# samtools/htslib

Hardware: NVIDIA H100
Metric: BGZF inflate + CRAM rANS decode GB/s at 1/2/4/8 H100 vs reference CPU (higher is better)
Workload: dtype u8

## Files before the change

### htslib_b200/csrc/bgzf_inflate.cu

```cuda
#include "hgpu_internal.h"

namespace {

constexpr int LIT_ROOT = 9, DST_ROOT = 8;
constexpr int LIT_TABLE = (1 << LIT_ROOT) + 856;
constexpr int DST_TABLE = (1 << DST_ROOT) + 512;
constexpr int CL_TABLE = 128;

enum : uint32_t { K_BAD = 0, K_LIT = 1, K_LEN = 2, K_SUB = 3, K_DIST = 4, K_EOB = 8 };
#define ENTRY(value, xb, kind, nbits) (((uint32_t)(value) << 16) | ((uint32_t)(xb) << 8) | ((uint32_t)(kind) << 4) | (uint32_t)(nbits))
constexpr uint32_t BAD_ENTRY = ENTRY(0, 0, K_BAD, 0);

struct InflateSmem {
    uint32_t lit[LIT_TABLE];
    uint32_t dst[DST_TABLE];
    union {
        struct {
            uint32_t cl[CL_TABLE];
            uint16_t code[320];
            uint8_t  lens[320];
            uint32_t count[16];
            uint32_t next[16];
            uint32_t sub_alloc;
        };
// ... 55 lines not shown
        b.w++;
        b.buf = v >> (8 * mis);
        b.cnt = 32 - 8 * (int)mis;
        b.avail -= b.cnt;
    }
}

__device__ __forceinline__ void bits_fill(Bits &b)
{
    if (b.cnt <= 32) {
        uint32_t v = b.w < b.wend ? (*b.w) : 0;
        b.w++;
        b.buf |= (uint64_t)v << b.cnt;
        b.cnt += 32;
        b.avail -= 32;
    }
}
__device__ __forceinline__ uint32_t bits_peek(const Bits &b, int n) { return (uint32_t)b.buf & ((1u << n) - 1u); }
__device__ __forceinline__ void bits_drop(Bits &b, int n) { b.buf >>= n; b.cnt -= n; }
__device__ __forceinline__ uint32_t bits_get(Bits &b, int n) { uint32_t v = bits_peek(b, n); bits_drop(b, n); return v; }
__device__ __forceinline__ bool bits_overrun(const Bits &b) { return b.avail + b.cnt < 0; }
__device__ __forceinline__ uint32_t bits_pos(const Bits &b) { return (uint32_t)((int64_t)b.end_bits - (b.avail + b.cnt)); }

template <int ROOT, int CAP, typename MakeEntry>
__device__ int build_table(InflateSmem &s, uint32_t *table, int n, bool allow_single, MakeEntry make)
{
    const uint32_t lane = hgpu_lane();
    __syncwarp();
    if (lane < 16) s.count[lane] = 0;
    for (int i = lane; i < CAP; i += 32) table[i] = BAD_ENTRY;
    if (lane == 0) s.sub_alloc = 1u << ROOT;
    __syncwarp();
    for (int i = lane; i < n; i += 32) atomicAdd(&s.count[s.lens[i]], 1u);
    __syncwarp();
    int maxlen = 0;
    int64_t left = 1;
    uint32_t code = 0;
    bool over = false;
    for (int l = 1; l <= 15; l++) {
        uint32_t c = s.count[l];
        left = (left << 1) - (int64_t)c;
        if (left < 0) over = true;
        if (c) maxlen = l;
        code = (code + (l > 1 ? s.count[l - 1] : 0)) << 1;
        if (l == 1) code = 0;
        if (lane == 0) s.next[l] = code;
    }
    if (over) return -1;
    if (maxlen == 0) return allow_single ? 0 : -1;
    if (left > 0 && !(allow_single && maxlen == 1)) return -1;
    __syncwarp();
    for (int base = 0; base < n; base += 32) {
        int i = base + lane;
        uint32_t l = i < n ? s.lens[i] : 0;
        uint32_t peers = __match_any_sync(0xffffffffu, l);
        uint32_t rank = __popc(peers & hgpu_lanemask_lt());
        if (l) s.code[i] = (uint16_t)(s.next[l] + rank);
        __syncwarp();
        if (l && rank + 1 == (uint32_t)__popc(peers)) s.next[l] += __popc(peers);
        __syncwarp();
    }
    for (int i = lane; i < n; i += 32) {
        uint32_t l = s.lens[i];
        if (!l) continue;
        uint32_t rev = __brev((uint32_t)s.code[i]) >> (32 - l);
        if (l <= ROOT) {
            uint32_t e = make(i, l);
            for (uint32_t k = rev; k < (1u << ROOT); k += 1u << l) table[k] = e;
        } else {
            atomicMax(&table[rev & ((1u << ROOT) - 1)], ENTRY(0, l - ROOT, K_SUB, ROOT) | 0x80000000u);
        }
    }
    __syncwarp();
    for (uint32_t k = lane; k < (1u << ROOT); k += 32) {
        uint32_t e = table[k];
        if (e & 0x80000000u) {
            uint32_t sub_bits = (e >> 8) & 0xff;
            uint32_t off = atomicAdd(&s.sub_alloc, 1u << sub_bits);
            table[k] = off + (1u << sub_bits) <= (uint32_t)CAP ? ENTRY(off, sub_bits, K_SUB, ROOT) : BAD_ENTRY;
        }
    }
    __syncwarp();
    if (s.sub_alloc > (uint32_t)CAP) return -1;
    for (int i = lane; i < n; i += 32) {
        uint32_t l = s.lens[i];
        if (l <= ROOT) continue;
        uint32_t rev = __brev((uint32_t)s.code[i]) >> (32 - l);
        uint32_t root = table[rev & ((1u << ROOT) - 1)];
        uint32_t off = root >> 16, sub_bits = (root >> 8) & 0xff;
        uint32_t e = make(i, l - ROOT);
        for (uint32_t k = rev >> ROOT; k < (1u << sub_bits); k += 1u << (l - ROOT)) table[off + k] = e;
    }
    __syncwarp();
    return 0;
}

__device__ __forceinline__ uint32_t lit_entry(int sym, uint32_t nbits)
{
    if (sym < 256) return ENTRY(sym, 0, K_LIT, nbits);
    if (sym == 256) return ENTRY(0, 0, K_EOB, nbits);
    if (sym > 285) return ENTRY(0, 0, K_BAD, nbits);
    return ENTRY(c_len_base[sym - 257], c_len_xtra[sym - 257], K_LEN, nbits);
}
__device__ __forceinline__ uint32_t dst_entry(int sym, uint32_t nbits)
{
    if (sym > 29) return ENTRY(0, 0, K_BAD, nbits);
    return ENTRY(c_dst_base[sym], c_dst_xtra[sym], K_DIST, nbits);
}
__device__ __forceinline__ uint32_t cl_entry(int sym, uint32_t nbits) { return ENTRY(sym, 0, K_LIT, nbits); }

template <int ROOT>
__device__ __forceinline__ uint32_t lookup(const uint32_t *table, Bits &b)
{
    uint32_t e = table[bits_peek(b, ROOT)];
    if (((e >> 4) & 15) == K_SUB) {
        bits_drop(b, ROOT);
        e = table[(e >> 16) + bits_peek(b, (e >> 8) & 0xff)];
    }
    bits_drop(b, e & 15);
    return e;
}

__device__ uint32_t multmodp(uint32_t a, uint32_t b)
{
    uint32_t p = 0;
    for (uint32_t m = 1u << 31; m; m >>= 1) {
        if (a & m) p ^= b;
        b = (b & 1) ? (b >> 1) ^ 0xEDB88320u : b >> 1;
    }
    return p;
}

__device__ uint32_t xpow_bytes(uint32_t nbytes)
{
    uint32_t p = 1u << 31;
    uint32_t sq = 1u << 23;
    while (nbytes) {
        if (nbytes & 1) p = multmodp(sq, p);
        sq = multmodp(sq, sq);
        nbytes >>= 1;
    }
    return p;
}

__global__ void crc_init_kernel()
{
    uint32_t i = threadIdx.x;
    uint32_t c = i;
    for (int k = 0; k < 8; k++) c = (c >> 1) ^ (0xEDB88320u & (0u - (c & 1)));
    g_crc_tab[0][i] = c;
    __syncthreads();
    uint32_t c1 = g_crc_tab[0][c & 0xff] ^ (c >> 8);
    g_crc_tab[1][i] = c1;
    uint32_t c2 = g_crc_tab[0][c1 & 0xff] ^ (c1 >> 8);
    g_crc_tab[2][i] = c2;
    uint32_t c3 = g_crc_tab[0][c2 & 0xff] ^ (c2 >> 8);
    g_crc_tab[3][i] = c3;
}

__global__ void crc_init2_kernel()
{
    const uint32_t i = threadIdx.x;
    for (int j = 0; j < 4; j++) {
        uint32_t v = g_crc_tab[j][i];
        for (int k = 0; k < 124; k++) v = g_crc_tab[0][v & 0xff] ^ (v >> 8);
        g_crc_tab2[j][i] = v;
    }
    g_xpow_lo[i] = xpow_bytes(i);
    g_xpow_hi[i] = xpow_bytes(256u * i);
    uint32_t v = 1u << 31;
    for (uint32_t k = 0; k < 8u * i; k++) v = (v & 0x80000000u) ? ((v ^ 0xEDB88320u) << 1) | 1u : v << 1;
    g_xinv_byte[i] = v;
}

__device__ uint32_t warp_crc32(const uint32_t (*tab)[256], const uint8_t *out, uint32_t n)
{
    const uint32_t lane = hgpu_lane();
    uint32_t c = n / 32, r = n % 32;
    uint32_t beg = lane == 0 ? 0 : r + lane * c;
    uint32_t len = lane == 0 ? c + r : c;
    uint32_t crc = 0xffffffffu;
    const uint8_t *p = out + beg, *e = p + len;
    while (p < e && (reinterpret_cast<uintptr_t>(p) & 15)) crc = tab[0][(crc ^ *p++) & 0xff] ^ (crc >> 8);
    if (e - p >= 16) {
        uint4 nx = *reinterpret_cast<const uint4 *>(p);
        while (e - p >= 16) {
            uint4 cur = nx;
            p += 16;
            if (e - p >= 16) nx = *reinterpret_cast<const uint4 *>(p);
            uint32_t wv[4] = {cur.x, cur.y, cur.z, cur.w};
#pragma unroll
            for (int k = 0; k < 4; k++) {
                crc ^= wv[k];
                crc = tab[3][crc & 0xff] ^ tab[2][(crc >> 8) & 0xff] ^ tab[1][(crc >> 16) & 0xff] ^ tab[0][crc >> 24];
            }
        }
    }
    while (p < e) crc = tab[0][(crc ^ *p++) & 0xff] ^ (crc >> 8);
    crc = ~crc;
    if (c == 0) return __shfl_sync(0xffffffffu, crc, 0);
    uint32_t xp = c < 65536u ? multmodp(g_xpow_hi[c >> 8], g_xpow_lo[c & 255u]) : xpow_bytes(c);
    for (int d = 1; d < 32; d <<= 1) {
        uint32_t right = __shfl_down_sync(0xffffffffu, crc, d);
        if ((lane & (2 * d - 1)) == 0) crc = multmodp(xp, crc) ^ right;
        xp = multmodp(xp, xp);
    }
    return __shfl_sync(0xffffffffu, crc, 0);
}

__device__ __forceinline__ uint32_t ld32_if(const uint8_t *a, bool c)
{
    uint32_t v;
    asm volatile("{\n\t.reg .pred q;\n\tsetp.ne.u32 q, %2, 0;\n\tmov.u32 %0, 0;\n\t@q ld.global.u32 %0, [%1];\n\t}" : "=r"(v) : "l"(a), "r"((uint32_t)c) : "memory");
    return v;
}
__device__ __forceinline__ void st32_if(uint8_t *a, uint32_t v, bool c)
{
    asm volatile("{\n\t.reg .pred q;\n\tsetp.ne.u32 q, %2, 0;\n\t@q st.global.u32 [%0], %1;\n\t}" :: "l"(a), "r"(v), "r"((uint32_t)c) : "memory");
}
__device__ __forceinline__ void st8_if(uint8_t *a, uint32_t v, bool c)
{
    asm volatile("{\n\t.reg .pred q;\n\tsetp.ne.u32 q, %2, 0;\n\t@q st.global.u8 [%0], %1;\n\t}" :: "l"(a), "r"(v), "r"((uint32_t)c) : "memory");
}

struct CrcCursor {
    const uint32_t *tab;
    const uint8_t *row0;
    uint32_t m0;
    uint32_t next;
    uint32_t acc;
};

__device__ __forceinline__ uint32_t crc_step4(const uint32_t *tab, uint32_t v)
{
    return tab[3 * 256 + (v & 0xff)] ^ tab[2 * 256 + ((v >> 8) & 0xff)] ^ tab[256 + ((v >> 16) & 0xff)] ^ tab[v >> 24];
}

__device__ __forceinline__ uint32_t ldg32(const uint8_t *a) { uint32_t v; asm volatile("ld.global.u32 %0, [%1];" : "=r"(v) : "l"(a) : "memory"); return v; }
__device__ __forceinline__ uint32_t ldg8(const uint8_t *a) { uint32_t v; asm volatile("ld.global.u8 %0, [%1];" : "=r"(v) : "l"(a) : "memory"); return v; }

__device__ __forceinline__ void crc_begin(CrcCursor &c, const uint32_t *tab, const uint8_t *out)
{
    const uintptr_t a = reinterpret_cast<uintptr_t>(out);
    c.tab = tab;
    c.row0 = reinterpret_cast<const uint8_t *>(a & ~(uintptr_t)127);
    c.m0 = (uint32_t)(a & 127);
    c.next = 0;
    c.acc = 0;
}

__device__ __forceinline__ uint32_t crc_edge_word(const CrcCursor &c, uint32_t q, uint32_t lim)
{
    uint32_t w = 0;
    if (q >= c.m0 && q + 4u <= lim) w = ldg32(c.row0 + q);
    else
        for (uint32_t i = 0; i < 4; i++)
            if (q + i >= c.m0 && q + i < lim) w |= ldg8(c.row0 + q + i) << (8 * i);
    const int32_t rel = (int32_t)c.m0 - (int32_t)q;
    if (rel > -4 && rel < 4) w ^= rel >= 0 ? 0xffffffffu << (8 * rel) : 0xffffffffu >> (-8 * rel);
    return w;
}

__device__ __forceinline__ void crc_absorb(CrcCursor &c, uint32_t r_end, uint32_t lim)
{
    const uint32_t l4 = 4u * hgpu_lane();
    const uint32_t *tab = c.tab;
    uint32_t r = c.next, acc = c.acc;
    const uint32_t ie = min(r_end, lim >> 7);
    for (; r < r_end && r < 2u; r++) acc = crc_step4(tab, acc ^ crc_edge_word(c, 128u * r + l4, lim));
    for (uint32_t r8 = r; r8 < ie; r8 += 8) {
        const uint8_t *p = c.row0 + 128u * r8 + l4;
        uint32_t w[8];
#pragma unroll
        for (uint32_t k = 0; k < 8; k++) w[k] = ld32_if(p + 128u * k, r8 + k < ie);
#pragma unroll
        for (uint32_t k = 0; k < 8; k++)
            if (r8 + k < ie) acc = crc_step4(tab, acc ^ w[k]);
    }
    r = max(r, ie);
    for (; r < r_end; r++) acc = crc_step4(tab, acc ^ crc_edge_word(c, 128u * r + l4, lim));
    c.acc = acc;
    c.next = r;
}

__device__ __forceinline__ void crc_advance(CrcCursor &c, uint32_t f)
{
    const uint32_t lim = c.m0 + f;
    if ((lim >> 7) > c.next) crc_absorb(c, lim >> 7, lim);
}

__device__ uint32_t crc_finish(CrcCursor &c, uint32_t n)
{
    const uint32_t lim = c.m0 + n;
    const uint32_t rows = (max(lim, c.m0 + 4u) + 127u) >> 7;
    crc_absorb(c, rows, lim);
    uint32_t s = multmodp(g_xinv_byte[4u * hgpu_lane()], c.acc);
#pragma unroll
    for (int d = 16; d; d >>= 1) s ^= __shfl_xor_sync(0xffffffffu, s, d);
    return ~multmodp(g_xinv_byte[128u * rows - lim], s);
}

__device__ __forceinline__ uint32_t low_mask(uint32_t n) { return n >= 32u ? 0xffffffffu : (1u << n) - 1u; }

struct WordSlot {
    uint32_t d;
    uint32_t lo, hi;
    uint32_t f;
};

__device__ __forceinline__ WordSlot load_slot(const uint8_t *ob, uint32_t inc, uint32_t wb, uint32_t u0, uint32_t ld,
                                              uint32_t slot, uint32_t T)
{
    const uint32_t lane = hgpu_lane();
    uint32_t k = 0;
#pragma unroll
    for (int st = 16; st >= 1; st >>= 1)
        if (__shfl_sync(0xffffffffu, inc, k + st - 1) <= slot) k += st;
    const uint32_t D = __shfl_sync(0xffffffffu, wb, k) + 4u * slot;
    const uint32_t a0 = __shfl_sync(0xffffffffu, u0, k), l_d = __shfl_sync(0xffffffffu, ld, k);
    const uint32_t kn = __shfl_down_sync(0xffffffffu, k, 1);
    const bool valid = slot < T;
    const uint32_t dist = l_d >> 16;
    const uint32_t a = max(D, a0), b = min(D + 4u, a0 + (l_d & 0xffffu));
    const int32_t S = (int32_t)(D - dist), S0 = S & ~3, sh = (S & 3) * 8;
    const bool from_next = lane < 31 && kn == k && slot + 1 < T;
    const bool need_lo = valid && S0 + 4 > (int32_t)(a - dist);
    const bool need_hi = valid && sh != 0 && S0 + 4 < (int32_t)(b - dist) && !from_next;
    WordSlot w;
    w.d = D;
    w.lo = ld32_if(ob + S0, need_lo);
    w.hi = ld32_if(ob + S0 + 4, need_hi);
    const uint32_t m = valid ? ((1u << (b - D)) - 1u) & ~((1u << (a - D)) - 1u) : 0u;
    w.f = m | (uint32_t)sh << 4 | (from_next ? 1u << 9 : 0u);
    return w;
}

__device__ __forceinline__ void store_slot(uint8_t *ob, const WordSlot &w)
{
    const uint32_t lo_next = __shfl_down_sync(0xffffffffu, w.lo, 1);
    const uint32_t v = __funnelshift_r(w.lo, (w.f >> 9) ? lo_next : w.hi, (w.f >> 4) & 31u);
    const uint32_t m = w.f & 15u;
    const bool part = m != 15u;
    st32_if(ob + w.d, v, !part);
    st8_if(ob + w.d, v, part && (m & 1u));
    st8_if(ob + w.d + 1, v >> 8, part && (m & 2u));
    st8_if(ob + w.d + 2, v >> 16, part && (m & 4u));
    st8_if(ob + w.d + 3, v >> 24, part && (m & 8u));
}

__device__ __forceinline__ void exec_batch(uint8_t *out, uint2 rec, uint32_t nrec)
{
    const uint32_t lane = hgpu_lane();
    const bool have = lane < nrec;
    const uint32_t len = have ? (rec.y & 0xffffu) : 0u, dist = rec.y >> 16;
    const uint32_t dst = have ? rec.x : 0xffffffffu;
    const uint32_t dst_end = have ? dst + len : 0xffffffffu;
    const bool ov = dist < len;
    const uint32_t src = dst - dist, src_end = ov ? dst : src + len;
    uint32_t dep = 0;
    const uint32_t dst0 = __shfl_sync(0xffffffffu, dst, 0);
    if (__any_sync(0xffffffffu, have && src_end > dst0)) {
        uint32_t j1 = 0, j2 = 0;
#pragma unroll
        for (int st = 16; st >= 1; st >>= 1) {
            uint32_t e = __shfl_sync(0xffffffffu, dst_end, j1 + st - 1);
            uint32_t d = __shfl_sync(0xffffffffu, dst, j2 + st - 1);
            if (e <= src) j1 += st;
            if (d < src_end) j2 += st;
        }
        if (have && j2 > j1) dep = low_mask(j2) & ~low_mask(j1) & hgpu_lanemask_lt();
    }
    const uint32_t mis = (uint32_t)reinterpret_cast<uintptr_t>(out) & 3u;
    uint8_t *ob = out - mis;
    const uint32_t u0 = dst + mis;
    const uint32_t nw = have && !ov ? ((u0 + len + 3u) >> 2) - (u0 >> 2) : 0u;
    uint32_t done = low_mask(nrec) ^ 0xffffffffu;
#ifdef HGPU_PROFILE
    if (lane == 0) atomicAdd(&g_prof[9], 1ull);
#endif
    while (done != 0xffffffffu) {
        const bool ready = !((done >> lane) & 1u) && (dep & ~done) == 0u;
        const uint32_t R = __ballot_sync(0xffffffffu, ready);
        const uint32_t Rov = __ballot_sync(0xffffffffu, ready && ov);
#ifdef HGPU_PROFILE
        if (lane == 0) { atomicAdd(&g_prof[8], 1ull); atomicAdd(&g_prof[11], (unsigned long long)__popc(Rov)); }
#endif
        const uint32_t cnt = ready ? nw : 0u;
        uint32_t inc = cnt;
#pragma unroll
        for (int d = 1; d < 32; d <<= 1) {
            const uint32_t t = __shfl_up_sync(0xffffffffu, inc, d);
            if (lane >= (uint32_t)d) inc += t;
        }
        const uint32_t T = __shfl_sync(0xffffffffu, inc, 31);
        const uint32_t wb = (u0 & ~3u) - 4u * (inc - cnt);
        if (T) {
            WordSlot cur = load_slot(ob, inc, wb, u0, rec.y, lane, T);
            for (uint32_t base = 0; base < T; base += 32) {
                WordSlot nxt = {0u, 0u, 0u, 0u};
                if (base + 32 < T) nxt = load_slot(ob, inc, wb, u0, rec.y, base + 32 + lane, T);
                store_slot(ob, cur);
                cur = nxt;
            }
        }
        __syncwarp();
        for (uint32_t m = Rov; m; m &= m - 1) {
            const int k = __ffs(m) - 1;
            const uint32_t d0 = __shfl_sync(0xffffffffu, dst, k), ln = __shfl_sync(0xffffffffu, len, k);
            const uint32_t di = __shfl_sync(0xffffffffu, dist, k);
            const uint32_t stepm = 32u % di;
            uint32_t r = lane % di;
            for (uint32_t i = lane; i < ln; i += 32) {
                out[d0 + i] = out[d0 - di + r];
                r += stepm;
                if (r >= di) r -= di;
            }
        }
        __syncwarp();
        done |= R;
    }
}

__device__ int decode_body_uniform(InflateSmem &s, Bits &b, uint8_t *out, uint32_t cap, uint32_t &o, CrcCursor &crc)
{
    const uint32_t lane = hgpu_lane();
    uint32_t pend = 0;
    for (;;) {
        bits_fill(b);
        uint32_t e = lookup<LIT_ROOT>(s.lit, b);
        uint32_t kind = (e >> 4) & 15;
        if (kind == K_LIT) {
            if (o >= cap) return HGPU_BGZF_ERR_SPACE;
            if (lane == 0) out[o] = (uint8_t)(e >> 16);
            o++;
            continue;
        }
        if (kind == K_EOB) break;
        if (kind != K_LEN) return HGPU_BGZF_ERR_ZLIB;
        uint32_t len = (e >> 16) + bits_get(b, (e >> 8) & 0xff);
        bits_fill(b);
        uint32_t d = lookup<DST_ROOT>(s.dst, b);
        if (((d >> 4) & 15) != K_DIST) return HGPU_BGZF_ERR_ZLIB;
        uint32_t dist = (d >> 16) + bits_get(b, (d >> 8) & 0xff);
        if (bits_overrun(b)) return HGPU_BGZF_ERR_ZLIB;
        if (dist > o) return HGPU_BGZF_ERR_ZLIB;
        if (o + len > cap) return HGPU_BGZF_ERR_SPACE;
        __syncwarp();
        if (lane == 0) s.rbuf[pend] = make_uint2(o, len | (dist << 16));
        o += len;
        if (++pend == 32) {
            __syncwarp();
            exec_batch(out, s.rbuf[lane], 32);
            pend = 0;
            crc_advance(crc, o);
        }
    }
    __syncwarp();
    if (pend) exec_batch(out, s.rbuf[lane], pend);
    __syncwarp();
    if (bits_overrun(b)) return HGPU_BGZF_ERR_ZLIB;
    return HGPU_OK;
}

struct LaneBits {
    const uint32_t *w;
    uint64_t buf;
    uint32_t nxt;
    int cnt;
    int lim;
};

__device__ __forceinline__ void lb_init(LaneBits &b, const uint32_t *wbase, const uint32_t *wend, uint32_t start, uint32_t end)
{
    uint32_t wi = start >> 5, off = start & 31;
    const uint32_t *p = wbase + wi;
    uint32_t w0 = p < wend ? p[0] : 0;
    b.nxt = p + 1 < wend ? p[1] : 0;
    b.w = p + 2;
    b.buf = w0 >> off;
    b.cnt = 32 - (int)off;
    b.lim = (int)((wi + 1) * 32) - (int)end;
}
__device__ __forceinline__ void lb_fill(LaneBits &b, const uint32_t *wend)
{
    if (b.cnt <= 32) {
        b.buf |= (uint64_t)b.nxt << b.cnt;
        b.cnt += 32;
        b.lim += 32;
        b.nxt = b.w < wend ? (*b.w) : 0;
        b.w++;
    }
}
__device__ __forceinline__ uint32_t lb_pos(const LaneBits &b, uint32_t end) { return (uint32_t)(b.lim + (int)end - b.cnt); }

template <int ROOT>
__device__ __forceinline__ uint32_t lb_lookup(const uint32_t *table, LaneBits &b)
{
    uint32_t e = table[(uint32_t)b.buf & ((1u << ROOT) - 1)];
    if (((e >> 4) & 15) == K_SUB) {
        b.buf >>= ROOT; b.cnt -= ROOT;
        e = table[(e >> 16) + ((uint32_t)b.buf & ((1u << ((e >> 8) & 0xff)) - 1))];
    }
    b.buf >>= (e & 15); b.cnt -= (int)(e & 15);
    return e;
}

enum : uint32_t { ST_RUN = 0, ST_EOB = 1, ST_BAD = 2 };

template <int EMIT>
__device__ __forceinline__ void lane_decode(const InflateSmem &s, const uint32_t *wbase, const uint32_t *wend,
                                            uint32_t start, uint32_t end, uint32_t &exitp, uint32_t &nout,
                                            uint32_t &nmatch, uint32_t &st, uint8_t *out, uint32_t obase,
                                            uint2 *mrec, uint32_t mbase, bool &bad_dist)
{
    LaneBits b;
    uint32_t n = 0, m = 0, status = ST_RUN;
    if (start >= end) { exitp = start; nout = 0; nmatch = 0; st = ST_RUN; return; }
    lb_init(b, wbase, wend, start, end);
    while (b.cnt > b.lim) {
        lb_fill(b, wend);
        uint32_t e = lb_lookup<LIT_ROOT>(s.lit, b);
        uint32_t kind = (e >> 4) & 15;
        if (kind == K_LIT) {
            if (EMIT) out[obase + n] = (uint8_t)(e >> 16);
            n++;
        } else if (kind == K_LEN) {
            uint32_t xb = (e >> 8) & 0xff;
            uint32_t len = (e >> 16) + ((uint32_t)b.buf & ((1u << xb) - 1));
            b.buf >>= xb; b.cnt -= (int)xb;
            lb_fill(b, wend);
            uint32_t d = lb_lookup<DST_ROOT>(s.dst, b);
            if (((d >> 4) & 15) != K_DIST) { status = ST_BAD; break; }
            uint32_t xd = (d >> 8) & 0xff;
            uint32_t dist = (d >> 16) + ((uint32_t)b.buf & ((1u << xd) - 1));
            b.buf >>= xd; b.cnt -= (int)xd;
            if (EMIT) {
                uint32_t dstpos = obase + n;
                if (dist > dstpos) bad_dist = true;
                mrec[mbase + m] = make_uint2(dstpos, len | (dist << 16));
            }
            n += len; m++;
        } else if (kind == K_EOB) { status = ST_EOB; break; }
        else { status = ST_BAD; break; }
    }
    exitp = lb_pos(b, end);
    nout = n; nmatch = m; st = status;
}

__device__ void run_matches(uint8_t *out, const uint2 *mrec, uint32_t total, CrcCursor &crc)
{
    const uint32_t lane = hgpu_lane();
    uint2 nx = lane < total ? mrec[lane] : make_uint2(0, 0);
    for (uint32_t base = 0; base < total; base += 32) {
        uint2 rec = nx;
        nx = base + 32 + lane < total ? mrec[base + 32 + lane] : make_uint2(0, 0);
        exec_batch(out, rec, total - base < 32u ? total - base : 32u);
        if (base + 32 < total) crc_advance(crc, __shfl_sync(0xffffffffu, nx.x, 0));
    }
    __syncwarp();
}

constexpr uint32_t PAR_MIN_BITS = 32 * 96;
constexpr uint32_t MREC_CAP = 65536 / 3 + 64;

__device__ int decode_body_parallel(InflateSmem &s, const uint32_t *wbase, const uint32_t *wend, uint32_t body,
                                    uint32_t total, uint8_t *out, uint32_t cap, uint32_t &o, uint2 *mrec,
                                    uint32_t &end_pos, CrcCursor &crc, Prof &pf, uint32_t mcap = MREC_CAP)
{
    const uint32_t lane = hgpu_lane();
    const uint32_t S = (total - body + 31) / 32;
    uint32_t start = body + lane * S;
    uint32_t end = lane == 31 ? total : min(total, body + (lane + 1) * S);
    if (start > total) start = total;
    uint32_t exitp = 0, n = 0, m = 0, st = ST_RUN;
    bool need = true, dummy = false;
    for (int round = 0; round < 34; round++) {
        if (need) lane_decode<0>(s, wbase, wend, start, end, exitp, n, m, st, nullptr, 0, nullptr, 0, dummy);
        uint32_t prev = __shfl_up_sync(0xffffffffu, exitp, 1);
        uint32_t ns = lane == 0 ? start : prev;
        need = ns != start;
        start = ns;
        if (!__any_sync(0xffffffffu, need)) break;
    }
    pf.mark(1);
    uint32_t eob = __ballot_sync(0xffffffffu, st == ST_EOB);
    uint32_t bad = __ballot_sync(0xffffffffu, st == ST_BAD);
    if (!eob) return HGPU_BGZF_ERR_ZLIB;
    uint32_t E = __ffs(eob) - 1;
    if (bad & ((2u << E) - 1u)) return HGPU_BGZF_ERR_ZLIB;
    uint32_t last = __shfl_sync(0xffffffffu, exitp, E);
    if (last > total) return HGPU_BGZF_ERR_ZLIB;
    if (lane > E) { n = 0; m = 0; }
    uint32_t on = n, mn = m;
#pragma unroll
    for (int d = 1; d < 32; d <<= 1) {
        uint32_t a = __shfl_up_sync(0xffffffffu, on, d), c = __shfl_up_sync(0xffffffffu, mn, d);
        if (lane >= (uint32_t)d) { on += a; mn += c; }
    }
    uint32_t tot_out = __shfl_sync(0xffffffffu, on, 31), tot_m = __shfl_sync(0xffffffffu, mn, 31);
    if ((uint64_t)o + tot_out > cap) return HGPU_BGZF_ERR_SPACE;
    if (tot_m > mcap) return HGPU_BGZF_ERR_ZLIB;
    bool bad_dist = false;
    if (lane <= E) {
        uint32_t e2, n2, m2, st2;
        lane_decode<1>(s, wbase, wend, start, end, e2, n2, m2, st2, out, o + on - n, mrec, mn - m, bad_dist);
    }
    if (__any_sync(0xffffffffu, bad_dist)) return HGPU_BGZF_ERR_ZLIB;
    __syncwarp();
    __threadfence_block();
    pf.mark(2);
    run_matches(out, mrec, tot_m, crc);
    pf.mark(3);
    o += tot_out;
    end_pos = last;
    return HGPU_OK;
}

__device__ int inflate_member(InflateSmem &s, const uint8_t *src, uint32_t slen, uint8_t *out, uint32_t cap,
                              uint32_t &olen, uint2 *mrec, CrcCursor &crc, Prof &pf, uint32_t mcap = MREC_CAP)
{
    const uint32_t lane = hgpu_lane();
    Bits b;
    bits_init(b, src, 0, slen);
    const uintptr_t a0 = reinterpret_cast<uintptr_t>(src);
    const uint32_t mis_bits = (uint32_t)(a0 & 3) * 8;
    const uint32_t *wbase = reinterpret_cast<const uint32_t *>(a0 - (a0 & 3));
    const uint32_t *wend = reinterpret_cast<const uint32_t *>((a0 + slen + 3) & ~(uintptr_t)3);
    const uint32_t total = mis_bits + slen * 8;
    uint32_t o = 0;
    for (;;) {
        bits_fill(b);
        uint32_t final = bits_get(b, 1), type = bits_get(b, 2);
        if (type == 0) {
            bits_drop(b, b.cnt & 7);
            bits_fill(b);
            uint32_t len = bits_get(b, 16);
            bits_fill(b);
            uint32_t nlen = bits_get(b, 16);
            if (bits_overrun(b)) return HGPU_BGZF_ERR_ZLIB;
            if ((len ^ 0xffffu) != nlen) return HGPU_BGZF_ERR_ZLIB;
            uint32_t pos = bits_pos(b) >> 3;
            if ((uint64_t)pos + len > slen) return HGPU_BGZF_ERR_ZLIB;
            if (o + len > cap) return HGPU_BGZF_ERR_SPACE;
            for (uint32_t i = lane; i < len; i += 32) out[o + i] = src[pos + i];
            o += len;
            bits_init(b, src, pos + len, slen);
            __syncwarp();
            crc_advance(crc, o);
        } else if (type == 1 || type == 2) {
            int rc;
            if (type == 1) {
                __syncwarp();
                for (int i = lane; i < 288; i += 32) s.lens[i] = i < 144 ? 8 : i < 256 ? 9 : i < 280 ? 7 : 8;
                __syncwarp();
                rc = build_table<LIT_ROOT, LIT_TABLE>(s, s.lit, 288, false, lit_entry);
                if (rc) return HGPU_BGZF_ERR_ZLIB;
                __syncwarp();
                for (int i = lane; i < 32; i += 32) s.lens[i] = 5;
                __syncwarp();
                rc = build_table<DST_ROOT, DST_TABLE>(s, s.dst, 32, false, dst_entry);
                if (rc) return HGPU_BGZF_ERR_ZLIB;
            } else {
                bits_fill(b);
                uint32_t hlit = bits_get(b, 5) + 257, hdist = bits_get(b, 5) + 1, hclen = bits_get(b, 4) + 4;
                if (hlit > 286 || hdist > 30) return HGPU_BGZF_ERR_ZLIB;
                __syncwarp();
                if (lane < 19) s.lens[lane] = 0;
                __syncwarp();
                for (uint32_t i = 0; i < hclen; i++) {
                    bits_fill(b);
                    uint32_t v = bits_get(b, 3);
                    if (lane == 0) s.lens[c_cl_order[i]] = (uint8_t)v;
                }
                if (bits_overrun(b)) return HGPU_BGZF_ERR_ZLIB;
                __syncwarp();
                rc = build_table<7, CL_TABLE>(s, s.cl, 19, false, cl_entry);
                if (rc) return HGPU_BGZF_ERR_ZLIB;
                uint32_t nsym = hlit + hdist, i = 0, prev = 0;
                while (i < nsym) {
                    bits_fill(b);
                    uint32_t e = s.cl[bits_peek(b, 7)];
                    if (((e >> 4) & 15) != K_LIT) return HGPU_BGZF_ERR_ZLIB;
                    bits_drop(b, e & 15);
                    uint32_t sym = e >> 16;
                    if (sym < 16) {
                        if (lane == 0) s.code[i] = (uint16_t)sym;
                        prev = sym; i++;
                    } else {
                        uint32_t rep, val = 0;
                        if (sym == 16) { if (i == 0) return HGPU_BGZF_ERR_ZLIB; val = prev; rep = 3 + bits_get(b, 2); }
                        else if (sym == 17) rep = 3 + bits_get(b, 3);
                        else rep = 11 + bits_get(b, 7);
                        if (i + rep > nsym) return HGPU_BGZF_ERR_ZLIB;
                        for (uint32_t k = lane; k < rep; k += 32) s.code[i + k] = (uint16_t)val;
                        i += rep;
                        prev = val;
                    }
                    if (bits_overrun(b)) return HGPU_BGZF_ERR_ZLIB;
                }
                __syncwarp();
                if (s.code[256] == 0) return HGPU_BGZF_ERR_ZLIB;
                uint32_t dl = lane < hdist ? s.code[hlit + lane] : 0;
                uint32_t ll[9];
#pragma unroll
                for (int k = 0; k < 9; k++) { uint32_t j = lane + 32 * k; ll[k] = j < hlit ? s.code[j] : 0; }
                __syncwarp();
#pragma unroll
                for (int k = 0; k < 9; k++) { uint32_t j = lane + 32 * k; if (j < 288) s.lens[j] = (uint8_t)ll[k]; }
                __syncwarp();
                rc = build_table<LIT_ROOT, LIT_TABLE>(s, s.lit, (int)hlit, true, lit_entry);
                if (rc) return HGPU_BGZF_ERR_ZLIB;
                __syncwarp();
                s.lens[lane] = (uint8_t)dl;
                __syncwarp();
                rc = build_table<DST_ROOT, DST_TABLE>(s, s.dst, (int)hdist, true, dst_entry);
                if (rc) return HGPU_BGZF_ERR_ZLIB;
            }
            __syncwarp();
            if (bits_overrun(b)) return HGPU_BGZF_ERR_ZLIB;
            uint32_t body = mis_bits + bits_pos(b);
            pf.mark(0);
            if (total - body >= PAR_MIN_BITS) {
                uint32_t end_pos = 0;
                rc = decode_body_parallel(s, wbase, wend, body, total, out, cap, o, mrec, end_pos, crc, pf, mcap);
                if (rc) return rc;
                uint32_t byte = (end_pos - mis_bits) >> 3, bit = (end_pos - mis_bits) & 7;
                bits_init(b, src, byte, slen);
                bits_fill(b);
                bits_drop(b, bit);
            } else {
                rc = decode_body_uniform(s, b, out, cap, o, crc);
                if (rc) return rc;
                pf.mark(5);
            }
            crc_advance(crc, o);
        } else
            return HGPU_BGZF_ERR_ZLIB;
        if (final) break;
    }
    olen = o;
    return HGPU_OK;
}

__device__ int check_header(const uint8_t *h)
{
    if (h[0] != 31 || h[1] != 139 || h[2] != 8) return -2;
    return ((h[3] & 4) && (h[10] | h[11] << 8) == 6 && h[12] == 'B' && h[13] == 'C' && (h[14] | h[15] << 8) == 2) ? 0 : -1;
}

#ifndef HGPU_INFLATE_WARPS
#define HGPU_INFLATE_WARPS 7
#endif
constexpr int INFLATE_WARPS = HGPU_INFLATE_WARPS;

#ifndef INFL_LB
#define INFL_LB 3
#endif
__global__ void __launch_bounds__(32 * INFLATE_WARPS, INFL_LB)
bgzf_inflate_kernel(const uint8_t *__restrict__ in, const uint64_t *__restrict__ in_off,
                    const uint32_t *__restrict__ in_len, uint32_t n, uint8_t *out,
                    const uint64_t *__restrict__ out_off, const uint32_t *__restrict__ out_cap,
                    uint32_t *out_len, int32_t *status, uint32_t *counter, uint2 *mrec_all)
{
    extern __shared__ __align__(16) uint8_t dyn_smem[];
    uint32_t *crc_tab = reinterpret_cast<uint32_t *>(dyn_smem);
    InflateSmem *smem_all = reinterpret_cast<InflateSmem *>(dyn_smem + 4096);
    for (int i = threadIdx.x; i < 1024; i += blockDim.x) crc_tab[i] = (&g_crc_tab2[0][0])[i];
    __syncthreads();
    InflateSmem &s = smem_all[threadIdx.x >> 5];
    uint2 *mrec = mrec_all + ((size_t)blockIdx.x * INFLATE_WARPS + (threadIdx.x >> 5)) * MREC_CAP;
    const uint32_t lane = hgpu_lane();
    for (;;) {
        uint32_t job = 0;
        if (lane == 0) job = atomicAdd(counter, 1u);
        job = __shfl_sync(0xffffffffu, job, 0);
        if (job >= n) break;
        const uint8_t *blk = in + in_off[job];
        uint32_t blen = in_len[job];
        uint8_t *dst = out + out_off[job];
        uint32_t cap = out_cap[job];
        if (cap > 65536u) cap = 65536u;
        int rc = HGPU_OK;
        uint32_t got = 0;
        if (blen < 26 || check_header(blk) != 0 || (uint32_t)(blk[16] | blk[17] << 8) + 1u != blen)
            rc = HGPU_BGZF_ERR_HEADER;
        else {
            Prof pf;
            pf.start();
            CrcCursor cc;
            crc_begin(cc, crc_tab, dst);
            rc = inflate_member(s, blk + 18, blen - 18, dst, cap, got, mrec, cc, pf);
            if (rc == HGPU_OK) {
                uint32_t want = blk[blen - 8] | blk[blen - 7] << 8 | blk[blen - 6] << 16 | (uint32_t)blk[blen - 5] << 24;
                pf.mark(6);
                uint32_t crc = crc_finish(cc, got);
                if (crc != want) rc = HGPU_BGZF_ERR_CRC;
                pf.mark(4);
            }
        }
        __syncwarp();
        if (lane == 0) { status[job] = rc; out_len[job] = rc == HGPU_OK ? got : 0; }
    }
}


constexpr uint32_t GZ_MREC = 32768 + 64;

__device__ int gzip_header_len(const uint8_t *h, uint32_t n)
{
    if (n < 18 || h[0] != 31 || h[1] != 139 || h[2] != 8 || (h[3] & 0xe0)) return -1;
    const uint32_t flg = h[3];
    uint32_t p = 10;
    if (flg & 4) { if (p + 2 > n) return -1; p += 2u + (h[p] | h[p + 1] << 8); }
    if (flg & 8) { while (p < n && h[p]) p++; p++; }
    if (flg & 16) { while (p < n && h[p]) p++; p++; }
    if (flg & 2) p += 2;
    return p + 8 <= n ? (int)p : -1;
}

__global__ void __launch_bounds__(32 * INFLATE_WARPS, INFL_LB)
gzip_inflate_kernel(const uint8_t *__restrict__ in, const uint64_t *__restrict__ in_off,
                    const uint32_t *__restrict__ in_len, uint32_t n, uint8_t *out,
                    const uint64_t *__restrict__ out_off, const uint32_t *__restrict__ out_cap,
                    uint32_t *out_len, int32_t *status, uint32_t *counter, uint2 *mrec_all)
{
    extern __shared__ __align__(16) uint8_t dyn_smem[];
    uint32_t *crc_tab = reinterpret_cast<uint32_t *>(dyn_smem);
    InflateSmem *smem_all = reinterpret_cast<InflateSmem *>(dyn_smem + 4096);
    for (int i = threadIdx.x; i < 1024; i += blockDim.x) crc_tab[i] = (&g_crc_tab2[0][0])[i];
    __syncthreads();
    InflateSmem &s = smem_all[threadIdx.x >> 5];
    uint2 *mrec = mrec_all + ((size_t)blockIdx.x * INFLATE_WARPS + (threadIdx.x >> 5)) * GZ_MREC;
    const uint32_t lane = hgpu_lane();
    for (;;) {
        uint32_t job = 0;
        if (lane == 0) job = atomicAdd(counter, 1u);
        job = __shfl_sync(0xffffffffu, job, 0);
        if (job >= n) break;
        const uint8_t *blk = in + in_off[job];
        const uint32_t blen = in_len[job];
        uint8_t *dst = out + out_off[job];
        const uint32_t cap = out_cap[job];
        int rc = HGPU_OK;
        uint32_t got = 0;
        const int hl = gzip_header_len(blk, blen);
        if (hl < 0) rc = HGPU_BGZF_ERR_HEADER;
        else {
            Prof pf;
            pf.start();
            CrcCursor cc;
            crc_begin(cc, crc_tab, dst);
            rc = inflate_member(s, blk + hl, blen - (uint32_t)hl, dst, cap, got, mrec, cc, pf, GZ_MREC);
            if (rc == HGPU_OK) {
                const uint8_t *f = blk + blen - 8;
                const uint32_t want = f[0] | f[1] << 8 | f[2] << 16 | (uint32_t)f[3] << 24;
                const uint32_t isize = f[4] | f[5] << 8 | f[6] << 16 | (uint32_t)f[7] << 24;
                const uint32_t crc = crc_finish(cc, got);
                if (crc != want || isize != got) rc = HGPU_BGZF_ERR_CRC;
            }
        }
        __syncwarp();
        if (lane == 0) { status[job] = rc; out_len[job] = rc == HGPU_OK ? got : 0; }
    }
}

__global__ void crc32_chunks_kernel(const uint8_t *buf, size_t len, size_t chunk, uint32_t *partial)
{
    size_t w = (size_t)blockIdx.x;
    size_t beg = w * chunk;
    if (beg >= len) return;
    size_t n = len - beg < chunk ? len - beg : chunk;
    uint32_t crc = warp_crc32(g_crc_tab, buf + beg, (uint32_t)n);
    if (hgpu_lane() == 0) partial[w] = crc;
}

__global__ void crc32_batch_kernel(const uint8_t *buf, const uint64_t *off, const uint32_t *len, uint32_t n, uint32_t *crc_out)
{
    const uint32_t i = blockIdx.x * (blockDim.x >> 5) + (threadIdx.x >> 5);
    if (i >= n) return;
    uint32_t crc = warp_crc32(g_crc_tab, buf + off[i], len[i]);
    if (hgpu_lane() == 0) crc_out[i] = crc;
}

bool g_crc_ready[64];

int ensure_crc_tables(hgpu_ctx *ctx, cudaStream_t st)
{
    if (g_crc_ready[ctx->device & 63]) return HGPU_OK;
    crc_init_kernel<<<1, 256, 0, st>>>();
    crc_init2_kernel<<<1, 256, 0, st>>>();
    hgpu_count_launch();
    if (hgpu_check(cudaGetLastError(), "crc init")) return HGPU_ERR_CUDA;
    if (hgpu_check(cudaStreamSynchronize(st), "crc init sync")) return HGPU_ERR_CUDA;
    g_crc_ready[ctx->device & 63] = true;
    return HGPU_OK;
}


constexpr uint32_t DEFL_HASH_BITS = 12;
constexpr uint32_t DEFL_MAX_IN = 0xff00 + 256;
constexpr uint32_t DEFL_TOK_CAP = 65536;

struct DeflateDyn {
    uint32_t freq[288 + 32];
    uint16_t code_ll[288], code_d[32];
    uint8_t  len_ll[288], len_d[32];
    uint16_t order[288];
    uint8_t  cl_sym[320], cl_ext[320];
    uint32_t cl_freq[19];
    uint16_t cl_code[19];
    uint8_t  cl_len[19];
    uint32_t n_cl;
    uint32_t w[576];
    uint16_t par[576];
    uint8_t  depth[576];
};
union DeflateSmem {
    uint16_t htab[1u << DEFL_HASH_BITS];
    DeflateDyn d;
};
static_assert(sizeof(DeflateDyn) <= (sizeof(uint16_t) << DEFL_HASH_BITS), "pass-2 tables fit the hash table's bytes");

__device__ __forceinline__ uint32_t fixed_lit_code(uint32_t sym, uint32_t &nbits)
{
    uint32_t code;
    if (sym < 144) { code = 0x30 + sym; nbits = 8; }
    else if (sym < 256) { code = 0x190 + (sym - 144); nbits = 9; }
    else if (sym < 280) { code = sym - 256; nbits = 7; }
    else { code = 0xc0 + (sym - 280); nbits = 8; }
    return __brev(code) >> (32 - nbits);
}

__device__ __forceinline__ uint32_t token_bits(uint32_t tok, uint32_t &nbits)
{
    if (!(tok >> 31)) return fixed_lit_code(tok & 0xff, nbits);
    uint32_t len = (tok & 0xff) + 3, dist = ((tok >> 8) & 0x7fff) + 1;
    uint32_t ls = 28;
    while (ls > 0 && c_len_base[ls] > len) ls--;
    uint32_t lx = c_len_xtra[ls], n1;
    uint32_t bits = fixed_lit_code(257 + ls, n1);
    bits |= (len - c_len_base[ls]) << n1; n1 += lx;
    uint32_t ds = 29;
    while (ds > 0 && c_dst_base[ds] > dist) ds--;
    uint32_t dx = c_dst_xtra[ds];
    bits |= (__brev(ds) >> 27) << n1; n1 += 5;
    bits |= (dist - c_dst_base[ds]) << n1; n1 += dx;
    nbits = n1;
    return bits;
}

__device__ __forceinline__ uint32_t len_symbol(uint32_t len) { uint32_t ls = 28; while (ls > 0 && c_len_base[ls] > len) ls--; return ls; }
__device__ __forceinline__ uint32_t dist_symbol(uint32_t dist) { uint32_t ds = 29; while (ds > 0 && c_dst_base[ds] > dist) ds--; return ds; }

__device__ void build_lengths(const uint32_t *freq, int n, int max_bits, uint8_t *len, uint16_t *order, uint32_t *w, uint16_t *par, uint8_t *depth)
{
    int used = 0;
    for (int i = 0; i < n; i++) { len[i] = 0; if (freq[i]) order[used++] = (uint16_t)i; }
    if (used == 0) return;
    if (used == 1) { len[order[0]] = 1; return; }
    for (int i = 1; i < used; i++) {
        const uint16_t v = order[i];
        const uint32_t fv = freq[v];
        int j = i - 1;
        while (j >= 0 && (freq[order[j]] > fv)) { order[j + 1] = order[j]; j--; }
        order[j + 1] = v;
    }
    for (int i = 0; i < used; i++) w[i] = freq[order[i]];
    int leaf = 0, inode = used, next = used;
    for (int k = 0; k < used - 1; k++) {
        int a, b;
        if (leaf < used && (inode >= next || w[leaf] <= w[inode])) a = leaf++; else a = inode++;
        if (leaf < used && (inode >= next || w[leaf] <= w[inode])) b = leaf++; else b = inode++;
        w[next] = w[a] + w[b];
        par[a] = par[b] = (uint16_t)next;
        next++;
    }
    const int root = next - 1;
    depth[root] = 0;
    for (int i = root - 1; i >= 0; i--) depth[i] = (uint8_t)(depth[par[i]] + 1);
    int cnt[32];
    for (int i = 0; i < 32; i++) cnt[i] = 0;
    for (int i = 0; i < used; i++) cnt[depth[i] > max_bits ? max_bits : depth[i]]++;
    uint32_t total = 0;
    for (int i = 1; i <= max_bits; i++) total += (uint32_t)cnt[i] << (max_bits - i);
    while (total > (1u << max_bits)) {
        cnt[max_bits]--;
        for (int i = max_bits - 1; i > 0; i--) if (cnt[i]) { cnt[i]--; cnt[i + 1] += 2; break; }
        total--;
    }
    int idx = used - 1;
    for (int l = 1; l <= max_bits; l++)
        for (int c = 0; c < cnt[l]; c++) len[order[idx--]] = (uint8_t)l;
}

__device__ void assign_codes(const uint8_t *len, int n, int max_bits, uint16_t *code)
{
    uint32_t bl_count[16], next_code[16];
    for (int i = 0; i < 16; i++) bl_count[i] = 0;
    for (int i = 0; i < n; i++) bl_count[len[i]]++;
    bl_count[0] = 0;
    uint32_t c = 0;
    for (int b = 1; b <= max_bits; b++) { c = (c + bl_count[b - 1]) << 1; next_code[b] = c; }
    for (int i = 0; i < n; i++) if (len[i]) code[i] = (uint16_t)(__brev(next_code[len[i]]++) >> (32 - len[i]));
}

__device__ __forceinline__ uint64_t token_bits_dyn(const DeflateDyn &d, uint32_t tok, uint32_t &nbits)
{
    if (!(tok >> 31)) { const uint32_t sym = tok & 0xff; nbits = d.len_ll[sym]; return d.code_ll[sym]; }
    const uint32_t len = (tok & 0xff) + 3, dist = ((tok >> 8) & 0x7fff) + 1;
    const uint32_t ls = len_symbol(len), ds = dist_symbol(dist);
    uint64_t bits = d.code_ll[257 + ls];
    uint32_t n1 = d.len_ll[257 + ls];
    bits |= (uint64_t)(len - c_len_base[ls]) << n1; n1 += c_len_xtra[ls];
    bits |= (uint64_t)d.code_d[ds] << n1; n1 += d.len_d[ds];
    bits |= (uint64_t)(dist - c_dst_base[ds]) << n1; n1 += c_dst_xtra[ds];
    nbits = n1;
    return bits;
}

__device__ __forceinline__ uint32_t ld4(const uint8_t *p) { return p[0] | (uint32_t)p[1] << 8 | (uint32_t)p[2] << 16 | (uint32_t)p[3] << 24; }

__device__ uint32_t deflate_block_warp(DeflateSmem &s, const uint32_t (*crc_tab)[256], const uint8_t *in, uint32_t n,
                                       int level, uint8_t *out, uint32_t *toks)
{
    const uint32_t lane = hgpu_lane();
    if (n > 65280u) return 0;
    const uint32_t crc = warp_crc32(crc_tab, in, n);
    uint32_t dlen = 0;
    bool stored = level == 0 || n < 16;
    if (!stored) {
        __syncwarp();
        for (uint32_t i = lane; i < (1u << DEFL_HASH_BITS); i += 32) s.htab[i] = 0;
        __syncwarp();
        uint32_t ntok = 0, covered = 0;
        for (uint32_t base = 0; base < n; base += 32) {
            const uint32_t p = base + lane;
            uint32_t mlen = 0, mdist = 0;
            const bool can = p + 4 <= n;
            uint32_t cand = 0, h = 0;
            if (can) { h = (ld4(in + p) * 2654435761u) >> (32 - DEFL_HASH_BITS); cand = s.htab[h]; }
            __syncwarp();
            if (can) s.htab[h] = (uint16_t)(p + 1);
            __syncwarp();
            if (can && p >= covered) {
                const uint32_t maxl = n - p < 258u ? n - p : 258u;
                if (cand && p + 1 - cand <= 32768u) {
                    const uint8_t *a = in + (cand - 1), *b = in + p;
                    uint32_t l = 0;
                    while (l < maxl && a[l] == b[l]) l++;
                    if (l >= 4) { mlen = l; mdist = p + 1 - cand; }
                }
                if (p >= 1) {
                    const uint8_t *b = in + p, *a1 = in + p - 1;
                    uint32_t l = 0;
                    while (l < maxl && a1[l] == b[l]) l++;
                    if (l >= 3 && l > mlen) { mlen = l; mdist = 1; }
                }
            }
            uint32_t cur = covered > base ? covered : base;
            const uint32_t cend = base + 32 < n ? base + 32 : n;
            uint32_t has = __ballot_sync(0xffffffffu, mlen != 0);
            while (cur < cend) {
                uint32_t rel = cur - base;
                uint32_t later = has & ~((1u << rel) - 1u);
                uint32_t nm = later ? (uint32_t)(__ffs(later) - 1) : 32u;
                uint32_t lit_end = base + nm < cend ? base + nm : cend;
                uint32_t nl = lit_end - cur;
                if (nl) {
                    if (p >= cur && p < lit_end && ntok + (p - cur) < DEFL_TOK_CAP) toks[ntok + (p - cur)] = in[p];
                    ntok += nl;
                    cur = lit_end;
                }
                if (nm < 32 && base + nm < cend) {
                    uint32_t ml = __shfl_sync(0xffffffffu, mlen, nm), md = __shfl_sync(0xffffffffu, mdist, nm);
                    if (level >= 4 && nm < 31 && base + nm + 1 < cend) {
                        const uint32_t ml1 = __shfl_sync(0xffffffffu, mlen, (nm + 1) & 31);
                        if (ml1 > ml + 1) { has &= ~(1u << nm); continue; }
                    }
                    if (lane == 0 && ntok < DEFL_TOK_CAP) toks[ntok] = 0x80000000u | (ml - 3) | ((md - 1) << 8);
                    ntok++;
                    cur = base + nm + ml;
                }
            }
            covered = cur;
        }
        __syncwarp();
        __threadfence_block();
        DeflateDyn &d = s.d;
        bool overflow = ntok > DEFL_TOK_CAP;
        for (uint32_t i = lane; i < 320; i += 32) d.freq[i] = 0;
        __syncwarp();
        uint32_t xbits = 0;
        for (uint32_t t = lane; t < ntok && !overflow; t += 32) {
            const uint32_t tok = toks[t];
            if (!(tok >> 31)) atomicAdd(&d.freq[tok & 0xff], 1u);
            else {
                const uint32_t ls = len_symbol((tok & 0xff) + 3), ds = dist_symbol(((tok >> 8) & 0x7fff) + 1);
                atomicAdd(&d.freq[257 + ls], 1u);
                atomicAdd(&d.freq[288 + ds], 1u);
                xbits += c_len_xtra[ls] + c_dst_xtra[ds];
            }
        }
        for (int dd = 16; dd > 0; dd >>= 1) xbits += __shfl_xor_sync(0xffffffffu, xbits, dd);
        __syncwarp();
        uint32_t use_dyn = 0, hlit = 257, hdist = 1, hclen = 4;
        if (lane == 0 && !overflow) {
            d.freq[256] = 1;
            uint64_t fixed_bits = 3 + xbits, dyn_bits = 3 + 14 + xbits;
            for (int i = 0; i < 288; i++) fixed_bits += (uint64_t)d.freq[i] * (i < 144 ? 8 : i < 256 ? 9 : i < 280 ? 7 : 8);
// ... 291 lines not shown
```

Before: 169.6.

## Checkpoint speculative decode for early resync and vectorize short-distance match runs

```diff
diff --git a/htslib_b200/csrc/bgzf_inflate.cu b/htslib_b200/csrc/bgzf_inflate.cu
--- a/htslib_b200/csrc/bgzf_inflate.cu
+++ b/htslib_b200/csrc/bgzf_inflate.cu
@@ -381,12 +381,30 @@
 
 __device__ __forceinline__ uint32_t low_mask(uint32_t n) { return n >= 32u ? 0xffffffffu : (1u << n) - 1u; }
 
+constexpr uint32_t RUN_MAX_DIST = 4;
+
+__device__ __forceinline__ uint32_t ld8_if(const uint8_t *a, bool c)
+{
+    uint32_t v;
+    asm volatile("{\n\t.reg .pred q;\n\tsetp.ne.u32 q, %2, 0;\n\tmov.u32 %0, 0;\n\t@q ld.global.u8 %0, [%1];\n\t}" : "=r"(v) : "l"(a), "r"((uint32_t)c) : "memory");
+    return v;
+}
+
 struct WordSlot {
     uint32_t d;
     uint32_t lo, hi;
     uint32_t f;
 };
 
+__device__ __forceinline__ uint32_t run_word(uint32_t p, uint32_t dist, uint32_t r)
+{
+    const uint32_t pat = p & low_mask(8u * dist);
+    const uint32_t lo = pat * (dist == 1u ? 0x01010101u : dist == 2u ? 0x00010001u : dist == 3u ? 0x01000001u : 1u);
+    const uint32_t hi = dist == 3u ? pat >> 8 | pat << 16 : lo;
+    return __funnelshift_r(lo, hi, 8u * r);
+}
+
+template <bool RUNS>
 __device__ __forceinline__ WordSlot load_slot(const uint8_t *ob, uint32_t inc, uint32_t wb, uint32_t u0, uint32_t ld,
                                               uint32_t slot, uint32_t T)
 {
@@ -400,24 +418,29 @@
     const uint32_t kn = __shfl_down_sync(0xffffffffu, k, 1);
     const bool valid = slot < T;
     const uint32_t dist = l_d >> 16;
+    const bool run = RUNS && dist < (l_d & 0xffffu);
     const uint32_t a = max(D, a0), b = min(D + 4u, a0 + (l_d & 0xffffu));
-    const int32_t S = (int32_t)(D - dist), S0 = S & ~3, sh = (S & 3) * 8;
-    const bool from_next = lane < 31 && kn == k && slot + 1 < T;
-    const bool need_lo = valid && S0 + 4 > (int32_t)(a - dist);
-    const bool need_hi = valid && sh != 0 && S0 + 4 < (int32_t)(b - dist) && !from_next;
+    const uint32_t sa = run ? a0 - dist : a - dist, sb = run ? a0 : b - dist;
+    const int32_t S = (int32_t)(run ? a0 - dist : D - dist), S0 = S & ~3, sh = (S & 3) * 8;
+    const bool from_next = lane < 31 && kn == k && slot + 1 < T && !run;
+    const bool need_lo = valid && S0 + 4 > (int32_t)sa;
+    const bool need_hi = valid && sh != 0 && S0 + 4 < (int32_t)sb && !from_next;
     WordSlot w;
     w.d = D;
     w.lo = ld32_if(ob + S0, need_lo);
     w.hi = ld32_if(ob + S0 + 4, need_hi);
     const uint32_t m = valid ? ((1u << (b - D)) - 1u) & ~((1u << (a - D)) - 1u) : 0u;
-    w.f = m | (uint32_t)sh << 4 | (from_next ? 1u << 9 : 0u);
+    const uint32_t t = D + 12u - a0, r = dist == 3u ? t % 3u : t & (dist - 1u);
+    w.f = m | (uint32_t)sh << 4 | (from_next ? 1u << 9 : 0u) | (run ? 1u << 10 | (dist - 1u) << 11 | r << 13 : 0u);
     return w;
 }
 
+template <bool RUNS>
 __device__ __forceinline__ void store_slot(uint8_t *ob, const WordSlot &w)
 {
     const uint32_t lo_next = __shfl_down_sync(0xffffffffu, w.lo, 1);
-    const uint32_t v = __funnelshift_r(w.lo, (w.f >> 9) ? lo_next : w.hi, (w.f >> 4) & 31u);
+    uint32_t v = __funnelshift_r(w.lo, ((w.f >> 9) & 1u) ? lo_next : w.hi, (w.f >> 4) & 31u);
+    if (RUNS && ((w.f >> 10) & 1u)) v = run_word(v, ((w.f >> 11) & 3u) + 1u, (w.f >> 13) & 3u);
     const uint32_t m = w.f & 15u;
     const bool part = m != 15u;
     st32_if(ob + w.d, v, !part);
@@ -425,6 +448,18 @@
     st8_if(ob + w.d + 1, v >> 8, part && (m & 2u));
     st8_if(ob + w.d + 2, v >> 16, part && (m & 4u));
     st8_if(ob + w.d + 3, v >> 24, part && (m & 8u));
+}
+
+template <bool RUNS>
+__device__ __forceinline__ void copy_words(uint8_t *ob, uint32_t inc, uint32_t wb, uint32_t u0, uint32_t ld, uint32_t T)
+{
+    WordSlot cur = load_slot<RUNS>(ob, inc, wb, u0, ld, hgpu_lane(), T);
+    for (uint32_t base = 0; base < T; base += 32) {
+        WordSlot nxt = {0u, 0u, 0u, 0u};
+        if (base + 32 < T) nxt = load_slot<RUNS>(ob, inc, wb, u0, ld, base + 32 + hgpu_lane(), T);
+        store_slot<RUNS>(ob, cur);
+        cur = nxt;
+    }
 }
 
 __device__ __forceinline__ void exec_batch(uint8_t *out, uint2 rec, uint32_t nrec)
@@ -452,7 +487,8 @@
     const uint32_t mis = (uint32_t)reinterpret_cast<uintptr_t>(out) & 3u;
     uint8_t *ob = out - mis;
     const uint32_t u0 = dst + mis;
-    const uint32_t nw = have && !ov ? ((u0 + len + 3u) >> 2) - (u0 >> 2) : 0u;
+    const bool long_run = ov && dist > RUN_MAX_DIST;
+    const uint32_t nw = have && !long_run ? ((u0 + len + 3u) >> 2) - (u0 >> 2) : 0u;
     uint32_t done = low_mask(nrec) ^ 0xffffffffu;
 #ifdef HGPU_PROFILE
     if (lane == 0) atomicAdd(&g_prof[9], 1ull);
@@ -460,9 +496,11 @@
     while (done != 0xffffffffu) {
         const bool ready = !((done >> lane) & 1u) && (dep & ~done) == 0u;
         const uint32_t R = __ballot_sync(0xffffffffu, ready);
-        const uint32_t Rov = __ballot_sync(0xffffffffu, ready && ov);
+        const uint32_t Rov = __ballot_sync(0xffffffffu, ready && long_run);
+        const bool runs = __any_sync(0xffffffffu, ready && ov && !long_run);
 #ifdef HGPU_PROFILE
-        if (lane == 0) { atomicAdd(&g_prof[8], 1ull); atomicAdd(&g_prof[11], (unsigned long long)__popc(Rov)); }
+        const uint32_t Rall = __ballot_sync(0xffffffffu, ready && ov);
+        if (lane == 0) { atomicAdd(&g_prof[8], 1ull); atomicAdd(&g_prof[11], (unsigned long long)__popc(Rall)); }
 #endif
         const uint32_t cnt = ready ? nw : 0u;
         uint32_t inc = cnt;
@@ -474,25 +512,37 @@
         const uint32_t T = __shfl_sync(0xffffffffu, inc, 31);
         const uint32_t wb = (u0 & ~3u) - 4u * (inc - cnt);
         if (T) {
-            WordSlot cur = load_slot(ob, inc, wb, u0, rec.y, lane, T);
-            for (uint32_t base = 0; base < T; base += 32) {
-                WordSlot nxt = {0u, 0u, 0u, 0u};
-                if (base + 32 < T) nxt = load_slot(ob, inc, wb, u0, rec.y, base + 32 + lane, T);
-                store_slot(ob, cur);
-                cur = nxt;
-            }
+            if (runs) copy_words<true>(ob, inc, wb, u0, rec.y, T);
+            else copy_words<false>(ob, inc, wb, u0, rec.y, T);
         }
         __syncwarp();
         for (uint32_t m = Rov; m; m &= m - 1) {
             const int k = __ffs(m) - 1;
             const uint32_t d0 = __shfl_sync(0xffffffffu, dst, k), ln = __shfl_sync(0xffffffffu, len, k);
             const uint32_t di = __shfl_sync(0xffffffffu, dist, k);
+            const uint8_t *per = out + d0 - di;
             const uint32_t stepm = 32u % di;
             uint32_t r = lane % di;
-            for (uint32_t i = lane; i < ln; i += 32) {
-                out[d0 + i] = out[d0 - di + r];
-                r += stepm;
-                if (r >= di) r -= di;
+#ifdef HGPU_PROFILE
+            if (lane == 0) atomicAdd(&g_prof[14], (unsigned long long)((ln + 31u) / 32u));
+#endif
+            if (di <= 32u) {
+                const uint32_t pb = ld8_if(per + lane, lane < di);
+                for (uint32_t i = lane; i - lane < ln; i += 32) {
+                    const uint32_t v = __shfl_sync(0xffffffffu, pb, r);
+                    st8_if(out + d0 + i, v, i < ln);
+                    r += stepm;
+                    if (r >= di) r -= di;
+                }
+            } else {
+                uint32_t v = ld8_if(per + r, lane < ln);
+                for (uint32_t i = lane; i < ln; i += 32) {
+                    r += stepm;
+                    if (r >= di) r -= di;
+                    const uint32_t nv = ld8_if(per + r, i + 32u < ln);
+                    st8_if(out + d0 + i, v, true);
+                    v = nv;
+                }
             }
         }
         __syncwarp();
@@ -586,17 +636,53 @@
 
 enum : uint32_t { ST_RUN = 0, ST_EOB = 1, ST_BAD = 2 };
 
-template <int EMIT>
+constexpr uint32_t CK_TOKENS = 32;
+constexpr uint32_t CK_STRIDE = 4;
+constexpr uint32_t CK_COUNTS = 32 * CK_TOKENS;
+constexpr uint32_t CK_RESULT = 2 * CK_COUNTS;
+constexpr uint32_t CK_WORDS = CK_RESULT + 4 * 32;
+
+enum : int { LD_ROUND0 = 0, LD_EMIT = 1, LD_RESYNC = 2 };
+
+template <int MODE>
 __device__ __forceinline__ void lane_decode(const InflateSmem &s, const uint32_t *wbase, const uint32_t *wend,
                                             uint32_t start, uint32_t end, uint32_t &exitp, uint32_t &nout,
                                             uint32_t &nmatch, uint32_t &st, uint8_t *out, uint32_t obase,
-                                            uint2 *mrec, uint32_t mbase, bool &bad_dist)
-{
+                                            uint2 *mrec, uint32_t mbase, bool &bad_dist,
+                                            uint32_t *ck, uint32_t &nck, uint32_t &iters)
+{
+    constexpr bool EMIT = MODE == LD_EMIT;
     LaneBits b;
-    uint32_t n = 0, m = 0, status = ST_RUN;
-    if (start >= end) { exitp = start; nout = 0; nmatch = 0; st = ST_RUN; return; }
+    uint32_t n = 0, m = 0, status = ST_RUN, it = 0;
+    if (MODE == LD_ROUND0) nck = 0;
+    if (start >= end) { exitp = start; nout = 0; nmatch = 0; st = ST_RUN; iters = 0; return; }
     lb_init(b, wbase, wend, start, end);
+    const uint32_t *cp = ck, *cp_end = ck + 32 * (MODE == LD_RESYNC ? nck : 0u);
+    uint32_t cur = cp < cp_end ? cp[0] : 0xffffffffu;
+    uint32_t nxt = cp + 32 < cp_end ? cp[32] : 0xffffffffu;
     while (b.cnt > b.lim) {
+        if (MODE == LD_ROUND0 && it < CK_STRIDE * CK_TOKENS && it % CK_STRIDE == 0) {
+            ck[32 * (it / CK_STRIDE)] = lb_pos(b, end);
+            ck[CK_COUNTS + 32 * (it / CK_STRIDE)] = n | m << 16;
+        }
+        if (MODE == LD_RESYNC && cp < cp_end) {
+            const uint32_t p = lb_pos(b, end);
+            while (cur < p && cp < cp_end) {
+                cp += 32;
+                cur = nxt;
+                nxt = cp + 32 < cp_end ? cp[32] : 0xffffffffu;
+            }
+            if (cur == p) {
+                const uint32_t c = cp[CK_COUNTS];
+                exitp = ck[CK_RESULT];
+                nout = n + ck[CK_RESULT + 32] - (c & 0xffffu);
+                nmatch = m + ck[CK_RESULT + 64] - (c >> 16);
+                st = ck[CK_RESULT + 96];
+                iters = it;
+                return;
+            }
+        }
+        it++;
         lb_fill(b, wend);
         uint32_t e = lb_lookup<LIT_ROOT>(s.lit, b);
         uint32_t kind = (e >> 4) & 15;
@@ -624,6 +710,11 @@
     }
     exitp = lb_pos(b, end);
     nout = n; nmatch = m; st = status;
+    iters = it;
+    if (MODE == LD_ROUND0) {
+        nck = min((it + CK_STRIDE - 1) / CK_STRIDE, CK_TOKENS);
+        ck[CK_RESULT] = exitp; ck[CK_RESULT + 32] = n; ck[CK_RESULT + 64] = m; ck[CK_RESULT + 96] = status;
+    }
 }
 
 __device__ void run_matches(uint8_t *out, const uint2 *mrec, uint32_t total, CrcCursor &crc)
@@ -641,6 +732,7 @@
 
 constexpr uint32_t PAR_MIN_BITS = 32 * 96;
 constexpr uint32_t MREC_CAP = 65536 / 3 + 64;
+static_assert(CK_WORDS <= 2 * MREC_CAP, "the re-sync checkpoints fit the match-record scratch");
 
 __device__ int decode_body_parallel(InflateSmem &s, const uint32_t *wbase, const uint32_t *wend, uint32_t body,
                                     uint32_t total, uint8_t *out, uint32_t cap, uint32_t &o, uint2 *mrec,
@@ -651,10 +743,21 @@
     uint32_t start = body + lane * S;
     uint32_t end = lane == 31 ? total : min(total, body + (lane + 1) * S);
     if (start > total) start = total;
-    uint32_t exitp = 0, n = 0, m = 0, st = ST_RUN;
+    uint32_t exitp = 0, n = 0, m = 0, st = ST_RUN, iters = 0;
     bool need = true, dummy = false;
+    uint32_t nck = 0;
+    uint32_t *ck = reinterpret_cast<uint32_t *>(mrec) + lane;
     for (int round = 0; round < 34; round++) {
-        if (need) lane_decode<0>(s, wbase, wend, start, end, exitp, n, m, st, nullptr, 0, nullptr, 0, dummy);
+        if (round == 0)
+            lane_decode<LD_ROUND0>(s, wbase, wend, start, end, exitp, n, m, st, nullptr, 0, nullptr, 0, dummy, ck, nck, iters);
+        else if (need)
+            lane_decode<LD_RESYNC>(s, wbase, wend, start, end, exitp, n, m, st, nullptr, 0, nullptr, 0, dummy, ck, nck, iters);
+        else
+            iters = 0;
+#ifdef HGPU_PROFILE
+        const uint32_t wi = __reduce_max_sync(0xffffffffu, iters);
+        if (lane == 0) atomicAdd(&g_prof[round == 0 ? 12 : 13], (unsigned long long)wi);
+#endif
         uint32_t prev = __shfl_up_sync(0xffffffffu, exitp, 1);
         uint32_t ns = lane == 0 ? start : prev;
         need = ns != start;
@@ -682,7 +785,7 @@
     bool bad_dist = false;
     if (lane <= E) {
         uint32_t e2, n2, m2, st2;
-        lane_decode<1>(s, wbase, wend, start, end, e2, n2, m2, st2, out, o + on - n, mrec, mn - m, bad_dist);
+        lane_decode<LD_EMIT>(s, wbase, wend, start, end, e2, n2, m2, st2, out, o + on - n, mrec, mn - m, bad_dist, ck, nck, iters);
     }
     if (__any_sync(0xffffffffu, bad_dist)) return HGPU_BGZF_ERR_ZLIB;
     __syncwarp();
@@ -884,6 +987,7 @@
 
 
 constexpr uint32_t GZ_MREC = 32768 + 64;
+static_assert(CK_WORDS <= 2 * GZ_MREC, "the re-sync checkpoints fit the match-record scratch");
 
 __device__ int gzip_header_len(const uint8_t *h, uint32_t n)
 {
```

New measurement: 175.3 (median of 6 runs). 3.4% higher.
